# arpitbansal297/Cold-Diffusion-Models

Hardware: NVIDIA H100
Metric: training-step images/sec (CelebA-128 deblur UNet, config 3) (higher is better)
Workload: dtype tf32

## Files before the change

cold_diffusion_models_b200/_lib.py:

```python
import ctypes as C
import os
import torch

_HERE = os.path.dirname(os.path.abspath(__file__))
LIB_PATH = os.path.join(_HERE, 'csrc', 'libcolddiff.so')
CD_MAX_TAPS = 16
CONV_SIMT, CONV_TC = 0, 1
ACT_NONE, ACT_GELU, ACT_GELU_BWD = 0, 1, 2


class ColdDiffError(RuntimeError):
    pass


if not os.path.exists(LIB_PATH):
    raise ImportError("libcolddiff.so not built (%s); run `python -c 'import __graft_entry__ as g; g.build()'`"
                      % LIB_PATH)
lib = C.CDLL(LIB_PATH)


class ConvSrc(C.Structure):
    _fields_ = [('src', C.c_void_p), ('ld', C.c_int32), ('C', C.c_int32), ('H', C.c_int32), ('W', C.c_int32),
                ('ntaps', C.c_int32), ('dy', C.c_int32 * CD_MAX_TAPS), ('dx', C.c_int32 * CD_MAX_TAPS),
                ('w', C.c_void_p), ('w_per_batch', C.c_int32)]


class ConvDesc(C.Structure):
    _fields_ = [('B', C.c_int32), ('Hg', C.c_int32), ('Wg', C.c_int32), ('sy', C.c_int32), ('sx', C.c_int32),
                ('Cout', C.c_int32), ('nsrc', C.c_int32), ('s', ConvSrc * 2),
                ('out', C.c_void_p), ('out_ld', C.c_int32), ('Ho', C.c_int32), ('Wo', C.c_int32),
                ('oys', C.c_int32), ('oxs', C.c_int32), ('oy0', C.c_int32), ('ox0', C.c_int32),
                ('bias', C.c_void_p), ('resid', C.c_void_p), ('resid_ld', C.c_int32),
                ('act', C.c_int32), ('round_tf32', C.c_int32),
                ('out2', C.c_void_p), ('out2_ld', C.c_int32),
                ('aux', C.c_void_p), ('aux_ld', C.c_int32)]




class RepackJob(C.Structure):
    _fields_ = [('src', C.c_void_p), ('dst', C.c_void_p), ('O', C.c_int32), ('I', C.c_int32), ('KH', C.c_int32), ('KW', C.c_int32),
                ('transposed_conv', C.c_int32), ('mode', C.c_int32), ('ntaps', C.c_int32), ('round_tf32', C.c_int32),
                ('ky', C.c_int32 * CD_MAX_TAPS), ('kx', C.c_int32 * CD_MAX_TAPS), ('block0', C.c_int32), ('nblocks', C.c_int32)]


lib.cd_version.restype = C.c_int
if os.environ.get('COLDDIFF_2CTA') in ('0', '1', '2'):
    lib.cd_conv_tc_set_2cta(int(os.environ['COLDDIFF_2CTA']))
lib.cd_last_error.argtypes = [C.c_char_p, C.c_size_t]
if os.environ.get('COLDDIFF_CONV_TWO_CTAS') in ('0', '64', '128', '192'):
    lib.cd_conv_tc_set_two_ctas(int(os.environ['COLDDIFF_CONV_TWO_CTAS']))
if os.environ.get('COLDDIFF_CONV_HALO') in ('0', '1', '2', '6', '8'):
    lib.cd_conv_tc_set_halo(int(os.environ['COLDDIFF_CONV_HALO']))
if os.environ.get('COLDDIFF_WGRAD_MODE') in ('0', '1', '8'):
    lib.cd_wgrad_tc_set_mode(int(os.environ['COLDDIFF_WGRAD_MODE']))
if os.environ.get('COLDDIFF_2CTA_BN') in ('0', '64', '128', '192'):
    lib.cd_conv_tc_set_2cta_bn(int(os.environ['COLDDIFF_2CTA_BN']))
if os.environ.get('COLDDIFF_CONV_STAGED_EPILOGUE') in ('0', '1', '2', '3'):
    lib.cd_conv_tc_set_staged_epilogue(int(os.environ['COLDDIFF_CONV_STAGED_EPILOGUE']))


def _check(rc, what):
    if rc != 0:
        buf = C.create_string_buffer(512)
        lib.cd_last_error(buf, 512)
        raise ColdDiffError("%s failed (%d): %s" % (what, rc, buf.value.decode()))


def stream():
    return C.c_void_p(torch.cuda.current_stream().cuda_stream)


def ptr(t):
    if t is None:
        return C.c_void_p(0)
    return C.c_void_p(t.data_ptr())


_LAUNCHES = {'cd_linattn_context_det': 2, 'cd_conv_wgrad': 2, 'cd_time_mlp_fwd': 2, 'cd_time_mlp2_fwd': 2, 'cd_version': 0, 'cd_last_error': 0}
_launch_count = 0


_PROF_SHAPE_ARGS = {'cd_dwconv7_fwd': (2, 3, 4, 5), 'cd_dwconv7_wgrad': (4, 5, 6, 7), 'cd_layernorm_bwd': (6, 7),
                    'cd_layernorm_fwd': (2, 3), 'cd_linattn_context_det': (2, 3), 'cd_linattn_bwd_kv': (2, 3)}
_prof = None
# ... 47 lines not shown
```

cold_diffusion_models_b200/csrc/conv_tc.cu:

```cuda
#include "tc_common.cuh"
#include "conv_epilogue.cuh"

namespace {

constexpr int kTileM = 128;
constexpr int kChunkK = 32;
constexpr int kABytes = kTileM * 128;
constexpr int kThreads = 288;
constexpr int kConsumerWarps = 8;

struct TcParams {
  int B, Hg, Wg;
  int TW, TH, TN;
  int tiles_x, tiles_y, tiles_n, tiles_co, total_tiles;
  int sy, sx;
  int Cout;
  int nsrc;
  int ntaps[2];
  int kchunks[2];
  int wpb[2];
  int8_t dy[2][CD_MAX_TAPS];
  int8_t dx[2][CD_MAX_TAPS];
  float* out; int out_ld; int Ho, Wo; int oys, oxs, oy0, ox0;
  const float* bias;
// ... 164 lines not shown
            asm volatile("bar.sync %0, 128;" :: "r"(bar_id) : "memory");
            const int w4 = tid >> 5;
            if (w4 < 2) {
              const int row = w4 * 32 + lane;
              uint32_t r[32];
#pragma unroll
              for (int e = 0; e < 32; ++e) r[e] = __float_as_uint(st[row * kEpiStageStride + e]);
              const long long pix = tile_pixel(p, tile, cw * 64 + row);
              cd_epilogue_staged32(r, st + w4 * 32 * kEpiStageStride, lane, pix < 0 ? 0 : pix, pix >= 0, co0 + c, p);
            }
          } else {
#pragma unroll
            for (int j = c / 8; j < c / 8 + 4; ++j) {
              if (pix0 >= 0) epi_pair(p, pix0, co0 + 8 * j + q2, acc[4 * j], acc[4 * j + 1]);
              if (pix1 >= 0) epi_pair(p, pix1, co0 + 8 * j + q2, acc[4 * j + 2], acc[4 * j + 3]);
            }
          }
        }
      } else {
#pragma unroll
        for (int j = 0; j < BN / 8; ++j) {
          if (pix0 >= 0) epi_pair(p, pix0, co0 + 8 * j + q2, acc[4 * j], acc[4 * j + 1]);
          if (pix1 >= 0) epi_pair(p, pix1, co0 + 8 * j + q2, acc[4 * j + 2], acc[4 * j + 3]);
        }
      }
    }
  }
  if constexpr (PAIR) cluster_sync();
}

constexpr int kRowsTW = 16, kRowsTH = kTileM / kRowsTW;
constexpr int kRowsBoxBytes = kRowsTW * (kRowsTH + 2) * 128;

template <int BN, int ABOXES, int STAGES, int CTAS>
__global__ void __launch_bounds__(kThreads, CTAS)
conv_rows_kernel(const __grid_constant__ CUtensorMap mapA0, const __grid_constant__ CUtensorMap mapA1,
                 const __grid_constant__ CUtensorMap mapB0, const __grid_constant__ CUtensorMap mapB1, const __grid_constant__ TcParams p) {
  constexpr int kBBytes = BN * 128;
  extern __shared__ uint8_t smem_raw[];
  const uint32_t raw_addr = smem_u32(smem_raw);
  uint8_t* smem = smem_raw + ((1024u - (raw_addr & 1023u)) & 1023u);
  uint8_t* abox = smem;
  uint8_t* wtile = smem + ABOXES * kRowsBoxBytes;
  uint64_t* bars = reinterpret_cast<uint64_t*>(wtile + STAGES * kBBytes);
  uint64_t* full_bar = bars;
  uint64_t* empty_bar = bars + STAGES;
  uint64_t* afull = bars + 2 * STAGES;
  uint64_t* aempty = bars + 2 * STAGES + ABOXES;
  static_assert(2 * (STAGES + ABOXES) * 8 <= 256, "barrier block is 256 bytes");
  const int warp = threadIdx.x >> 5, lane = threadIdx.x & 31, wg = threadIdx.x >> 7;
  if (threadIdx.x == 0) {
    for (int i = 0; i < STAGES; ++i) { mbar_init(&full_bar[i], 1); mbar_init(&empty_bar[i], kConsumerWarps); }
    for (int i = 0; i < ABOXES; ++i) { mbar_init(&afull[i], 1); mbar_init(&aempty[i], kConsumerWarps); }
    asm volatile("fence.mbarrier_init.release.cluster;" ::: "memory");
  }
  __syncthreads();

  if (warp == kConsumerWarps) {
    if (elect_one()) {
      uint32_t stage = 0, ph = 0, ai = 0, aph = 0;
      for (int tile = blockIdx.x; tile < p.total_tiles; tile += gridDim.x) {
        const int co0 = (tile % p.tiles_co) * BN;
        int mt = tile / p.tiles_co;
        const int x0 = (mt % p.tiles_x) * kRowsTW; mt /= p.tiles_x;
        const int y0 = (mt % p.tiles_y) * kRowsTH;
        const int n = mt / p.tiles_y;
        for (int s = 0; s < p.nsrc; ++s) {
          const CUtensorMap* mA = s ? &mapA1 : &mapA0;
          const CUtensorMap* mB = s ? &mapB1 : &mapB0;
          for (int kc = 0; kc < p.kchunks[s]; ++kc) {
            for (int b = 0, i = 0; b < p.nbox[s]; ++b) {
              mbar_wait(&aempty[ai], aph ^ 1u);
              mbar_expect_tx(&afull[ai], kRowsBoxBytes);
              tma_load_4d(smem_u32(abox + ai * kRowsBoxBytes), mA, &afull[ai], kc * kChunkK, x0 + p.boxdx[s][b], y0 - 1, n);
              if (++ai == ABOXES) { ai = 0; aph ^= 1u; }
              for (; i < p.boxend[s][b]; ++i) {
                mbar_wait(&empty_bar[stage], ph ^ 1u);
                mbar_expect_tx(&full_bar[stage], kBBytes);
                tma_load_3d(smem_u32(wtile + stage * kBBytes), mB, &full_bar[stage], kc * kChunkK, co0, p.taporder[s][i]);
                if (++stage == STAGES) { stage = 0; ph ^= 1u; }
              }
            }
          }
        }
      }
    }
    __syncwarp();
    return;
  }

  const int tid = threadIdx.x & 127;
  const int rl = (tid >> 5) * 16 + (lane >> 2);
  const int q2 = (lane & 3) * 2;
  auto release = [&](uint64_t* bar) { __syncwarp(); if (lane == 0) mbar_arrive(bar); };
  float acc[BN / 2];
  uint32_t stage = 0, ph = 0, ai = 0, aph = 0;
  for (int tile = blockIdx.x; tile < p.total_tiles; tile += gridDim.x) {
    int k = 0;
    uint32_t prev = 0, prev_a = 0;
    for (int s = 0; s < p.nsrc; ++s) {
      for (int kc = 0; kc < p.kchunks[s]; ++kc) {
        for (int b = 0, i = 0; b < p.nbox[s]; ++b) {
          mbar_wait(&afull[ai], aph);
          const uint32_t abase = smem_u32(abox + ai * kRowsBoxBytes) + wg * (kABytes / 2);
          for (const int i0 = i; i < p.boxend[s][b]; ++i, ++k) {
            mbar_wait(&full_bar[stage], ph);
            wgmma_fence();
            const uint64_t da = make_kmajor_sw128_desc(abase + p.tapoff[s][i]);
            const uint64_t db = make_kmajor_sw128_desc(smem_u32(wtile + stage * kBBytes));
#pragma unroll
            for (int kk = 0; kk < 4; ++kk)
              wgmma_tf32<BN>(acc, da + uint64_t(kk * 2), db + uint64_t(kk * 2), (k | kk) != 0 ? 1u : 0u);
            wgmma_commit();
            wgmma_wait<1>();
            if (k > 0) release(&empty_bar[prev]);
            if (k > 0 && i == i0) release(&aempty[prev_a]);
            prev = stage;
            if (++stage == STAGES) { stage = 0; ph ^= 1u; }
          }
          prev_a = ai;
          if (++ai == ABOXES) { ai = 0; aph ^= 1u; }
        }
      }
    }
    wgmma_wait<0>();
    if (k > 0) { release(&empty_bar[prev]); release(&aempty[prev_a]); }

    const int co0 = (tile % p.tiles_co) * BN;
    int mt = tile / p.tiles_co;
    const int x0 = (mt % p.tiles_x) * kRowsTW; mt /= p.tiles_x;
    const int y0 = (mt % p.tiles_y) * kRowsTH;
    const int n = mt / p.tiles_y;
#pragma unroll
    for (int h = 0; h < 2; ++h) {
      const int m = wg * 64 + rl + 8 * h;
      const int gx = x0 + m % kRowsTW, gy = y0 + m / kRowsTW;
      if (gx >= p.Wg || gy >= p.Hg) continue;
      const long long pix = (static_cast<long long>(n) * p.Ho + (gy * p.oys + p.oy0)) * p.Wo + (gx * p.oxs + p.ox0);
#pragma unroll
      for (int j = 0; j < BN / 8; ++j) epi_pair(p, pix, co0 + 8 * j + q2, acc[4 * j + 2 * h], acc[4 * j + 2 * h + 1]);
    }
  }
}


int g_tf32_map_dtype = 1;

template <auto Kernel, size_t kSmem, int CTAS, bool PAIR = false>
int launch_persistent(const CUtensorMap* maps, const TcParams& p, cudaStream_t st) {
  static_assert(kSmem <= 232448, "dynamic shared memory of one CTA (227 KB)");
  static_assert(CTAS == 1 || 2 * (kSmem + 1024) <= 233472, "two CTAs per SM must fit the 228 KB of shared memory");
  CD_CUDA(smem_limit_once<Kernel>(kSmem));
  if constexpr (PAIR) {
    const int units = p.tiles_co * ((p.total_tiles / p.tiles_co + 1) / 2), slots = cd_num_sms() / 2;
    cudaLaunchConfig_t cfg = {};
    cudaLaunchAttribute attr[1];
    attr[0].id = cudaLaunchAttributeClusterDimension;
    attr[0].val.clusterDim.x = 2; attr[0].val.clusterDim.y = 1; attr[0].val.clusterDim.z = 1;
    cfg.gridDim = dim3(2 * (units < slots ? units : slots)); cfg.blockDim = dim3(kThreads);
    cfg.dynamicSmemBytes = kSmem; cfg.stream = st; cfg.attrs = attr; cfg.numAttrs = 1;
    CD_CUDA(cudaLaunchKernelEx(&cfg, Kernel, maps[0], maps[1], maps[2], maps[3], p));
  } else {
    const int slots = cd_num_sms() * CTAS;
    const int grid = p.total_tiles < slots ? p.total_tiles : slots;
    Kernel<<<grid, kThreads, kSmem, st>>>(maps[0], maps[1], maps[2], maps[3], p);
  }
  CD_LAUNCH_CHECK();
  return 0;
}

template <int BN, int STAGES, bool STG = false, bool F16 = false, int CTAS = 1, bool PAIR = false>
int launch(const CUtensorMap* maps, const TcParams& p, cudaStream_t st) {
  constexpr size_t smem = size_t(STAGES) * (kABytes + BN * 128) + 1024 + 256 + (STG ? sizeof(float) * 2 * 64 * kEpiStageStride : 0);
  return launch_persistent<conv_tc_kernel<BN, STAGES, STG, F16, CTAS, PAIR>, smem, CTAS, PAIR>(maps, p, st);
}

template <int BN, int ABOXES, int STAGES, int CTAS = 1>
int launch_rows(const CUtensorMap* maps, const TcParams& p, cudaStream_t st) {
  constexpr size_t smem = size_t(ABOXES) * kRowsBoxBytes + size_t(STAGES) * BN * 128 + 1024 + 256;
  return launch_persistent<conv_rows_kernel<BN, ABOXES, STAGES, CTAS>, smem, CTAS>(maps, p, st);
}

bool operands_ok(const CdConvDesc* d, int chunk_elems, int esz, bool report) {
#define TC_CHECK(cond, ...) do { if (!(cond)) { if (report) cd_set_error(__VA_ARGS__); return false; } } while (0)
  TC_CHECK(d->nsrc >= 1 && d->nsrc <= 2, "conv_tc: nsrc must be 1 or 2");
  TC_CHECK(d->act != CD_ACT_GELU_BWD || (d->aux && (reinterpret_cast<uintptr_t>(d->aux) & 15) == 0 && d->aux_ld % 4 == 0), "conv_tc: GELU_BWD needs an aligned aux");
  TC_CHECK((reinterpret_cast<uintptr_t>(d->out) & 15) == 0 && d->out_ld % 4 == 0, "conv_tc: out must be 16B aligned");
  TC_CHECK(!d->resid || ((reinterpret_cast<uintptr_t>(d->resid) & 15) == 0 && d->resid_ld % 4 == 0), "conv_tc: resid alignment");
  TC_CHECK(!d->out2 || ((reinterpret_cast<uintptr_t>(d->out2) & 15) == 0 && d->out2_ld % 4 == 0), "conv_tc: out2 alignment");
  TC_CHECK(!d->bias || (reinterpret_cast<uintptr_t>(d->bias) & 15) == 0, "conv_tc: bias alignment");
  for (int s = 0; s < d->nsrc; ++s) {
    const CdConvSrc& cs = d->s[s];
    TC_CHECK(cs.C % chunk_elems == 0 && cs.C > 0, "conv_tc: source channels %d not a multiple of %d", cs.C, chunk_elems);
    TC_CHECK(cs.ntaps >= 1 && cs.ntaps <= CD_MAX_TAPS, "conv_tc: bad ntaps");
    TC_CHECK((reinterpret_cast<uintptr_t>(cs.src) & 15) == 0 && (cs.ld * esz) % 16 == 0, "conv_tc: src must be 16B aligned");
    TC_CHECK((reinterpret_cast<uintptr_t>(cs.w) & 15) == 0, "conv_tc: weights must be 16B aligned");
  }
#undef TC_CHECK
  return true;
}

TcParams desc_params(const CdConvDesc* d, int chunk_elems) {
  TcParams p{};
  p.B = d->B; p.Hg = d->Hg; p.Wg = d->Wg; p.sy = d->sy; p.sx = d->sx; p.Cout = d->Cout; p.nsrc = d->nsrc;
  for (int s = 0; s < 2; ++s) {
    const CdConvSrc& cs = d->s[s < d->nsrc ? s : 0];
    p.ntaps[s] = cs.ntaps; p.kchunks[s] = cs.C / chunk_elems; p.wpb[s] = cs.w_per_batch;
    for (int t = 0; t < cs.ntaps; ++t) { p.dy[s][t] = (int8_t)cs.dy[t]; p.dx[s][t] = (int8_t)cs.dx[t]; }
  }
  p.out = d->out; p.out_ld = d->out_ld; p.Ho = d->Ho; p.Wo = d->Wo;
  p.oys = d->oys; p.oxs = d->oxs; p.oy0 = d->oy0; p.ox0 = d->ox0;
  p.bias = d->bias; p.resid = d->resid; p.resid_ld = d->resid_ld; p.act = d->act; p.round_tf32 = d->round_tf32;
  p.out2 = d->out2; p.out2_ld = d->out2_ld; p.aux = d->aux; p.aux_ld = d->aux_ld;
  return p;
}
// ... 3 lines not shown
extern "C" int cd_conv_tc_set_tf32_maps(int enable) { g_tf32_map_dtype = enable ? 1 : 0; return 0; }

static int g_use_2cta = 0;
extern "C" int cd_conv_tc_set_2cta(int mode) { g_use_2cta = mode; return 0; }
static int g_2cta_bn = 0;
extern "C" int cd_conv_tc_set_2cta_bn(int mask) { g_2cta_bn = mask & (128 | 64); return 0; }
static int g_use_halo = 0;
extern "C" int cd_conv_tc_set_halo(int enable) { g_use_halo = enable; return 0; }
static int g_ctas2 = 128 | 64;
extern "C" int cd_conv_tc_set_two_ctas(int mask) { g_ctas2 = mask & (128 | 64); return 0; }
static int g_epi_staged = 0;
constexpr int kStagedMaxKIters = 16;
constexpr int kStagedMidKIters = 48;
extern "C" int cd_conv_tc_set_staged_epilogue(int mode) { g_epi_staged = mode; return 0; }

static double tc_cost(long long m_tiles, int Cout, int BN, int sms, bool pair = false) {
  if (pair) {
    const long long tiles = ((m_tiles + 1) / 2) * (Cout / 256), slots = sms / 2;
    return double((tiles + slots - 1) / slots) * 256.0;
  }
  const long long tiles = m_tiles * ((Cout + BN - 1) / BN);
  const double rate = BN == 256 ? 0.92 : (BN == 128 ? 0.75 : 0.40);
  return double((tiles + sms - 1) / sms) * BN / rate;
}

static int conv_fwd_tc_impl(const CdConvDesc* d, cudaStream_t st, bool f16);
int cd_conv_fwd_tc(const CdConvDesc* d, cudaStream_t st) { return conv_fwd_tc_impl(d, st, false); }

extern "C" int cd_conv_fwd_f16_probe(const CdConvDesc* d, void* stream) {
  CD_REQUIRE(d != nullptr && d->nsrc >= 1 && d->nsrc <= 2, "cd_conv_fwd_f16_probe: bad descriptor");
  return conv_fwd_tc_impl(d, static_cast<cudaStream_t>(stream), true);
}

static int conv_fwd_rows(const CdConvDesc* d, cudaStream_t st, bool by_shape);

static int conv_fwd_tc_impl(const CdConvDesc* d, cudaStream_t st, bool f16) {
  if (!f16 && g_epi_staged == 0) {
    if ((g_use_halo == 0 && !g_use_2cta) || g_use_halo == 1 || g_use_halo == 2 || g_use_halo == 6) {
      const int r = conv_fwd_rows(d, st, g_use_halo == 0);
      if (r <= 0) return r;
    }
  }
  const CUtensorMapDataType dt = f16 ? CU_TENSOR_MAP_DATA_TYPE_FLOAT16 : (g_tf32_map_dtype ? CU_TENSOR_MAP_DATA_TYPE_TFLOAT32 : CU_TENSOR_MAP_DATA_TYPE_FLOAT32);
  const int esz = map_elem_bytes(dt), chunk_elems = 128 / esz;
  if (!operands_ok(d, chunk_elems, esz, true)) return -1;
  TcParams p = desc_params(d, chunk_elems);
  if (d->Wg >= 128) {
    CD_REQUIRE(d->Wg % 128 == 0, "conv_tc: Wg >= 128 must be a multiple of 128 (got %d)", d->Wg);
    p.TW = 128; p.TH = 1; p.TN = 1;
  } else {
    CD_REQUIRE(is_pow2(d->Wg), "conv_tc: Wg < 128 must be a power of two (got %d)", d->Wg);
    p.TW = d->Wg;
    int th = 128 / p.TW;
    if (th > d->Hg) th = d->Hg;
    CD_REQUIRE(is_pow2(th) && d->Hg % th == 0, "conv_tc: unsupported Hg %d for Wg %d", d->Hg, d->Wg);
    p.TH = th; p.TN = 128 / (p.TW * p.TH);
  }
  CD_REQUIRE(p.TW * d->sx <= 256 && p.TH * d->sy <= 256, "conv_tc: strided box too large");
  p.tiles_x = d->Wg / p.TW; p.tiles_y = d->Hg / p.TH; p.tiles_n = cd_cdiv(d->B, p.TN);
  int BN = (d->Cout % 256 == 0) ? 256 : (d->Cout > 64 ? 128 : 64);
  int kiters_host = 0;
  for (int s = 0; s < d->nsrc; ++s) kiters_host += d->s[s].ntaps * (d->s[s].C / chunk_elems);
  const bool staged = !f16 &&
                      ( g_epi_staged == 2 || (g_epi_staged == 1 && kiters_host <= kStagedMaxKIters) ||
                      (g_epi_staged == 3 && kiters_host <= kStagedMidKIters));
  bool pair = false;
  const long long mt = static_cast<long long>(p.tiles_x) * p.tiles_y * p.tiles_n;
  const int sms = cd_num_sms();
  if (BN == 256) {
    double best = tc_cost(mt, d->Cout, 256, sms);
    if (tc_cost(mt, d->Cout, 128, sms) < best) { BN = 128; best = tc_cost(mt, d->Cout, 128, sms); }
    if (!f16 && !staged && g_use_2cta && mt >= 2 && (g_use_2cta == 2 || tc_cost(mt, d->Cout, 256, sms, true) < best)) {
// ... 6 lines not shown
  p.total_tiles = p.tiles_x * p.tiles_y * p.tiles_n * p.tiles_co;

  CUtensorMap maps[4];
  for (int s = 0; s < 2; ++s) {
    const CdConvSrc& cs = d->s[s < d->nsrc ? s : 0];
    CD_REQUIRE(!cs.w_per_batch || p.TN == 1, "conv_tc: per-batch weights need >=128 pixels per image");
    if (!encode_nhwc(&maps[s], dt, cs.src, cs.ld, cs.C, cs.W, cs.H, d->B, 1, 1, 0, 0, p.TW * d->sx, p.TH * d->sy, p.TN, d->sx, d->sy,
                     s ? "A1" : "A0") ||
        !encode_weights(&maps[2 + s], dt, cs.w, cs.C, d->Cout, cs.ntaps * (cs.w_per_batch ? d->B : 1), pair ? BN / 2 : BN,
                        s ? "B1" : "B0"))
      return -1;
  }
  if (f16) {
    if (BN == 256) return launch<256, 4, false, true>(maps, p, st);
    if (BN == 128) return launch<128, 6, false, true>(maps, p, st);
    return launch<64, 8, false, true>(maps, p, st);
  }
  if (staged) {
    if (BN == 256) return launch<256, 3, true>(maps, p, st);
    if (BN == 128) return launch<128, 4, true>(maps, p, st);
    return launch<64, 6, true>(maps, p, st);
  }
  if (pair) {
    if (BN == 256) return launch<256, 4, false, false, 1, true>(maps, p, st);
    if (BN == 128) return launch<128, 6, false, false, 1, true>(maps, p, st);
    return launch<64, 8, false, false, 1, true>(maps, p, st);
  }
  const int ctas2 = p.total_tiles > sms ? g_ctas2 : 0;
  if (BN == 256) return launch<256, 4>(maps, p, st);
  if (BN == 128) return (ctas2 & 128) ? launch<128, 3, false, false, 2>(maps, p, st) : launch<128, 6>(maps, p, st);
  return (ctas2 & 64) ? launch<64, 4, false, false, 2>(maps, p, st) : launch<64, 8>(maps, p, st);
}

static int conv_fwd_rows(const CdConvDesc* d, cudaStream_t st, bool by_shape) {
  if (d->sy != 1 || d->sx != 1 || !operands_ok(d, kChunkK, 4, false)) return 1;
  for (int s = 0; s < d->nsrc; ++s) {
    const CdConvSrc& cs = d->s[s];
    if (cs.w_per_batch || cs.W != d->Wg || cs.H != d->Hg) return 1;
    for (int t = 0; t < cs.ntaps; ++t) if (cs.dy[t] < -1 || cs.dy[t] > 1 || cs.dx[t] < -1 || cs.dx[t] > 1) return 1;
  }
  TcParams p = desc_params(d, kChunkK);
  p.TW = kRowsTW; p.TH = kRowsTH; p.TN = 1;
  p.tiles_x = cd_cdiv(d->Wg, kRowsTW); p.tiles_y = cd_cdiv(d->Hg, kRowsTH); p.tiles_n = d->B;
  const int BN = d->Cout > 64 ? 128 : 64;
  p.tiles_co = cd_cdiv(d->Cout, BN);
  p.total_tiles = p.tiles_x * p.tiles_y * p.tiles_n * p.tiles_co;
  const int sms = cd_num_sms();
  if (by_shape && p.total_tiles <= sms) return 1;
  const CUtensorMapDataType dt = g_tf32_map_dtype ? CU_TENSOR_MAP_DATA_TYPE_TFLOAT32 : CU_TENSOR_MAP_DATA_TYPE_FLOAT32;
  CUtensorMap maps[4];
  for (int s = 0; s < 2; ++s) {
    const CdConvSrc& cs = d->s[s < d->nsrc ? s : 0];
    int i = 0;
    for (int dx = -1; dx <= 1; ++dx) {
      const int i0 = i;
      for (int t = 0; t < cs.ntaps; ++t)
        if (cs.dx[t] == dx) { p.taporder[s][i] = (int8_t)t; p.tapoff[s][i] = (cs.dy[t] + 1) * kRowsTW * 128; ++i; }
      if (i > i0) { p.boxdx[s][p.nbox[s]] = (int8_t)dx; p.boxend[s][p.nbox[s]] = (int8_t)i; ++p.nbox[s]; }
    }
    if (s == 0 && cs.ntaps < 3 * p.nbox[0]) return 1;
    if (!encode_nhwc(&maps[s], dt, cs.src, cs.ld, cs.C, cs.W, cs.H, d->B, 1, 1, 0, 0, kRowsTW, kRowsTH + 2, 1, 1, 1,
                     s ? "rows A1" : "rows A0") ||
        !encode_weights(&maps[2 + s], dt, cs.w, cs.C, d->Cout, cs.ntaps, BN, s ? "rows B1" : "rows B0"))
      return -1;
  }
  const int ctas2 = p.total_tiles > sms ? g_ctas2 : 0;
  if (BN == 128) return (ctas2 & 128) ? launch_rows<128, 3, 3, 2>(maps, p, st) : launch_rows<128, 6, 4>(maps, p, st);
  return (ctas2 & 64) ? launch_rows<64, 3, 6, 2>(maps, p, st) : launch_rows<64, 6, 8>(maps, p, st);
}
```

cold_diffusion_models_b200/csrc/dwconv_tma.cu:

```cuda
#include "tc_common.cuh"

namespace {

constexpr int kTY = 16;
constexpr int kWTX = 16;

__device__ __forceinline__ float* align128(uint8_t* raw) {
  return reinterpret_cast<float*>(raw + ((128u - (smem_u32(raw) & 127u)) & 127u));
}
__device__ __forceinline__ void fence_proxy_async() { asm volatile("fence.proxy.async.shared::cta;" ::: "memory"); }

template <int TX>
__global__ void __launch_bounds__(32 * kTY, 1)
dwconv7_tma_kernel(const __grid_constant__ CUtensorMap mapX, int B, int H, int W, int C,
                   const float* __restrict__ wdw, const float* __restrict__ bdw, const float* __restrict__ cond, int cond_ld,
                   float* __restrict__ out, int out_ld, int flip, const float* __restrict__ addend, int addend_ld) {
  extern __shared__ uint8_t dw_smem_raw[];
  float* xsp = align128(dw_smem_raw);
  __shared__ uint64_t full[2];
  constexpr int TY = kTY, XW = TX + 6, YH = TY + 6;
  constexpr int tile_floats = YH * XW * 32;
  const int lane = threadIdx.x & 31, ry = threadIdx.x >> 5;
  const int tiles_x = W / TX, tiles_y = H / TY;
  const int ntiles = B * tiles_x * tiles_y;
  const int total = (C / 32) * ntiles;

  if (threadIdx.x == 0) {
    mbar_init(&full[0], 1); mbar_init(&full[1], 1);
    asm volatile("fence.mbarrier_init.release.cluster;" ::: "memory");
  }
  __syncthreads();

  auto issue = [&](int item, int bi) {
    const int slab = item / ntiles, t = item - slab * ntiles;
    const int tx = t % tiles_x, ty = (t / tiles_x) % tiles_y, b = t / (tiles_x * tiles_y);
    fence_proxy_async();
    mbar_expect_tx(&full[bi], tile_floats * 4);
    tma_load_4d(smem_u32(xsp + bi * tile_floats), &mapX, &full[bi], slab * 32, tx * TX - 3, ty * TY - 3, b);
  };

  int item = blockIdx.x;
  if (item >= total) return;
  int bufi = 0;
// ... 182 lines not shown
```

cold_diffusion_models_b200/csrc/tc_common.cuh:

```cuda
#pragma once
#include "cd_common.cuh"

namespace {

__device__ __forceinline__ uint32_t smem_u32(const void* p) {
  return static_cast<uint32_t>(__cvta_generic_to_shared(p));
}
__device__ __forceinline__ uint32_t elect_one() {
  uint32_t pred = 0;
  asm volatile(
      "{\n"
      ".reg .pred px;\n"
      "elect.sync _|px, 0xffffffff;\n"
      "@px mov.s32 %0, 1;\n"
      "}\n" : "+r"(pred));
  return pred;
}
__device__ __forceinline__ void mbar_init(uint64_t* bar, uint32_t count) {
  asm volatile("mbarrier.init.shared::cta.b64 [%0], %1;" :: "r"(smem_u32(bar)), "r"(count) : "memory");
}
__device__ __forceinline__ void mbar_expect_tx(uint64_t* bar, uint32_t bytes) {
  asm volatile("mbarrier.arrive.expect_tx.shared::cta.b64 _, [%0], %1;"
               :: "r"(smem_u32(bar)), "r"(bytes) : "memory");
}
__device__ __forceinline__ void mbar_arrive(uint64_t* bar) {
  asm volatile("mbarrier.arrive.shared::cta.b64 _, [%0];" :: "r"(smem_u32(bar)) : "memory");
}
__device__ __forceinline__ void mbar_wait(uint64_t* bar, uint32_t parity) {
  asm volatile(
      "{\n"
      ".reg .pred p;\n"
      "WAIT_%=:\n"
      "mbarrier.try_wait.parity.shared::cta.b64 p, [%0], %1;\n"
      "@p bra DONE_%=;\n"
      "bra WAIT_%=;\n"
      "DONE_%=:\n"
      "}\n" :: "r"(smem_u32(bar)), "r"(parity) : "memory");
}
__device__ __forceinline__ void tma_load_4d(uint32_t dst, const CUtensorMap* map, uint64_t* bar,
                                            int c0, int c1, int c2, int c3) {
  asm volatile(
      "cp.async.bulk.tensor.4d.shared::cluster.global.mbarrier::complete_tx::bytes"
      " [%0], [%1, {%3, %4, %5, %6}], [%2];"
      :: "r"(dst), "l"(reinterpret_cast<uint64_t>(map)), "r"(smem_u32(bar)),
         "r"(c0), "r"(c1), "r"(c2), "r"(c3) : "memory");
}
__device__ __forceinline__ void tma_load_3d(uint32_t dst, const CUtensorMap* map, uint64_t* bar,
                                            int c0, int c1, int c2) {
  asm volatile(
      "cp.async.bulk.tensor.3d.shared::cluster.global.mbarrier::complete_tx::bytes"
      " [%0], [%1, {%3, %4, %5}], [%2];"
      :: "r"(dst), "l"(reinterpret_cast<uint64_t>(map)), "r"(smem_u32(bar)),
         "r"(c0), "r"(c1), "r"(c2) : "memory");
}
__device__ __forceinline__ uint64_t make_kmajor_sw128_desc(uint32_t saddr) {
  uint64_t d = 0;
  d |= static_cast<uint64_t>((saddr >> 4) & 0x3FFFu);
  d |= static_cast<uint64_t>(1) << 16;
  d |= static_cast<uint64_t>(1024 >> 4) << 32;
  d |= static_cast<uint64_t>(1) << 62;
  return d;
}
__device__ __forceinline__ void wgmma_fence() { asm volatile("wgmma.fence.sync.aligned;" ::: "memory"); }
__device__ __forceinline__ void wgmma_commit() { asm volatile("wgmma.commit_group.sync.aligned;" ::: "memory"); }
template <int N>
__device__ __forceinline__ void wgmma_wait() { asm volatile("wgmma.wait_group.sync.aligned %0;" :: "n"(N) : "memory"); }

template <int N> __device__ __forceinline__ void wgmma_tf32(float (&d)[N / 2], uint64_t da, uint64_t db, uint32_t acc);
template <int N> __device__ __forceinline__ void wgmma_f16(float (&d)[N / 2], uint64_t da, uint64_t db, uint32_t acc);
template <> __device__ __forceinline__ void wgmma_tf32<64>(float (&d)[32], uint64_t da, uint64_t db, uint32_t acc) {
  asm volatile(
      "{\n.reg .pred p;\nsetp.ne.b32 p, %34, 0;\n"
      "wgmma.mma_async.sync.aligned.m64n64k8.f32.tf32.tf32 {%0, %1, %2, %3, %4, %5, %6, %7, %8, %9, %10, %11, %12, %13, %14, %15, %16, %17, %18, %19, %20, %21, %22, %23, %24, %25, %26, %27, %28, %29, %30, %31}, %32, %33, p, 1, 1;\n}\n"
      : "+f"(d[0]), "+f"(d[1]), "+f"(d[2]), "+f"(d[3]), "+f"(d[4]), "+f"(d[5]), "+f"(d[6]), "+f"(d[7]), "+f"(d[8]), "+f"(d[9]), "+f"(d[10]), "+f"(d[11]), "+f"(d[12]), "+f"(d[13]), "+f"(d[14]), "+f"(d[15]), "+f"(d[16]), "+f"(d[17]), "+f"(d[18]), "+f"(d[19]), "+f"(d[20]), "+f"(d[21]), "+f"(d[22]), "+f"(d[23]), "+f"(d[24]), "+f"(d[25]), "+f"(d[26]), "+f"(d[27]), "+f"(d[28]), "+f"(d[29]), "+f"(d[30]), "+f"(d[31])
      : "l"(da), "l"(db), "r"(acc));
}
template <> __device__ __forceinline__ void wgmma_tf32<128>(float (&d)[64], uint64_t da, uint64_t db, uint32_t acc) {
  asm volatile(
      "{\n.reg .pred p;\nsetp.ne.b32 p, %66, 0;\n"
      "wgmma.mma_async.sync.aligned.m64n128k8.f32.tf32.tf32 {%0, %1, %2, %3, %4, %5, %6, %7, %8, %9, %10, %11, %12, %13, %14, %15, %16, %17, %18, %19, %20, %21, %22, %23, %24, %25, %26, %27, %28, %29, %30, %31, %32, %33, %34, %35, %36, %37, %38, %39, %40, %41, %42, %43, %44, %45, %46, %47, %48, %49, %50, %51, %52, %53, %54, %55, %56, %57, %58, %59, %60, %61, %62, %63}, %64, %65, p, 1, 1;\n}\n"
      : "+f"(d[0]), "+f"(d[1]), "+f"(d[2]), "+f"(d[3]), "+f"(d[4]), "+f"(d[5]), "+f"(d[6]), "+f"(d[7]), "+f"(d[8]), "+f"(d[9]), "+f"(d[10]), "+f"(d[11]), "+f"(d[12]), "+f"(d[13]), "+f"(d[14]), "+f"(d[15]), "+f"(d[16]), "+f"(d[17]), "+f"(d[18]), "+f"(d[19]), "+f"(d[20]), "+f"(d[21]), "+f"(d[22]), "+f"(d[23]), "+f"(d[24]), "+f"(d[25]), "+f"(d[26]), "+f"(d[27]), "+f"(d[28]), "+f"(d[29]), "+f"(d[30]), "+f"(d[31]), "+f"(d[32]), "+f"(d[33]), "+f"(d[34]), "+f"(d[35]), "+f"(d[36]), "+f"(d[37]), "+f"(d[38]), "+f"(d[39]), "+f"(d[40]), "+f"(d[41]), "+f"(d[42]), "+f"(d[43]), "+f"(d[44]), "+f"(d[45]), "+f"(d[46]), "+f"(d[47]), "+f"(d[48]), "+f"(d[49]), "+f"(d[50]), "+f"(d[51]), "+f"(d[52]), "+f"(d[53]), "+f"(d[54]), "+f"(d[55]), "+f"(d[56]), "+f"(d[57]), "+f"(d[58]), "+f"(d[59]), "+f"(d[60]), "+f"(d[61]), "+f"(d[62]), "+f"(d[63])
      : "l"(da), "l"(db), "r"(acc));
}
template <> __device__ __forceinline__ void wgmma_tf32<256>(float (&d)[128], uint64_t da, uint64_t db, uint32_t acc) {
  asm volatile(
      "{\n.reg .pred p;\nsetp.ne.b32 p, %130, 0;\n"
      "wgmma.mma_async.sync.aligned.m64n256k8.f32.tf32.tf32 {%0, %1, %2, %3, %4, %5, %6, %7, %8, %9, %10, %11, %12, %13, %14, %15, %16, %17, %18, %19, %20, %21, %22, %23, %24, %25, %26, %27, %28, %29, %30, %31, %32, %33, %34, %35, %36, %37, %38, %39, %40, %41, %42, %43, %44, %45, %46, %47, %48, %49, %50, %51, %52, %53, %54, %55, %56, %57, %58, %59, %60, %61, %62, %63, %64, %65, %66, %67, %68, %69, %70, %71, %72, %73, %74, %75, %76, %77, %78, %79, %80, %81, %82, %83, %84, %85, %86, %87, %88, %89, %90, %91, %92, %93, %94, %95, %96, %97, %98, %99, %100, %101, %102, %103, %104, %105, %106, %107, %108, %109, %110, %111, %112, %113, %114, %115, %116, %117, %118, %119, %120, %121, %122, %123, %124, %125, %126, %127}, %128, %129, p, 1, 1;\n}\n"
// ... 129 lines not shown
```

Before: 622.1.

## Add 256-pixel rows conv kernel with two consumer warpgroups and TMA-store epilogue

Adds a conv_rows256 kernel that uses a taller 16x16 pixel tile, so each loaded halo box is shared by two consumer warpgroups, each issuing two 64-row wgmma accumulators. It uses setmaxnreg to shift registers from the producer warpgroup to the consumers, and writes results through swizzled shared-memory staging and TMA bulk stores. The kernel is chosen by default when the taller tiling still gives enough tiles to fill the SMs and the output is unstrided. This is meant to cut A-operand reload traffic per output and the cost of scattered global stores, at the price of fewer tiles (possible SM underfill) and one CTA per SM. The producer loop is refactored into a shared helper.

```diff
diff --git a/cold_diffusion_models_b200/_lib.py b/cold_diffusion_models_b200/_lib.py
--- a/cold_diffusion_models_b200/_lib.py
+++ b/cold_diffusion_models_b200/_lib.py
@@ -50,7 +50,7 @@
 lib.cd_last_error.argtypes = [C.c_char_p, C.c_size_t]
 if os.environ.get('COLDDIFF_CONV_TWO_CTAS') in ('0', '64', '128', '192'):
     lib.cd_conv_tc_set_two_ctas(int(os.environ['COLDDIFF_CONV_TWO_CTAS']))
-if os.environ.get('COLDDIFF_CONV_HALO') in ('0', '1', '2', '6', '8'):
+if os.environ.get('COLDDIFF_CONV_HALO') in ('0', '1', '2', '4', '6', '8'):
     lib.cd_conv_tc_set_halo(int(os.environ['COLDDIFF_CONV_HALO']))
 if os.environ.get('COLDDIFF_WGRAD_MODE') in ('0', '1', '8'):
     lib.cd_wgrad_tc_set_mode(int(os.environ['COLDDIFF_WGRAD_MODE']))
diff --git a/cold_diffusion_models_b200/csrc/conv_tc.cu b/cold_diffusion_models_b200/csrc/conv_tc.cu
--- a/cold_diffusion_models_b200/csrc/conv_tc.cu
+++ b/cold_diffusion_models_b200/csrc/conv_tc.cu
@@ -220,6 +220,43 @@
 constexpr int kRowsTW = 16, kRowsTH = kTileM / kRowsTW;
 constexpr int kRowsBoxBytes = kRowsTW * (kRowsTH + 2) * 128;
 
+template <int BN, int TH, int ABOXES, int STAGES>
+__device__ __forceinline__ void rows_producer(const CUtensorMap& mapA0, const CUtensorMap& mapA1, const CUtensorMap& mapB0,
+                                              const CUtensorMap& mapB1, const TcParams& p, uint8_t* abox, uint8_t* wtile,
+                                              uint64_t* afull, uint64_t* aempty, uint64_t* full_bar, uint64_t* empty_bar) {
+  constexpr int kBBytes = BN * 128;
+  constexpr int kBoxBytes = kRowsTW * (TH + 2) * 128;
+  if (elect_one()) {
+    uint32_t stage = 0, ph = 0, ai = 0, aph = 0;
+    for (int tile = blockIdx.x; tile < p.total_tiles; tile += gridDim.x) {
+      const int co0 = (tile % p.tiles_co) * BN;
+      int mt = tile / p.tiles_co;
+      const int x0 = (mt % p.tiles_x) * kRowsTW; mt /= p.tiles_x;
+      const int y0 = (mt % p.tiles_y) * TH;
+      const int n = mt / p.tiles_y;
+      for (int s = 0; s < p.nsrc; ++s) {
+        const CUtensorMap* mA = s ? &mapA1 : &mapA0;
+        const CUtensorMap* mB = s ? &mapB1 : &mapB0;
+        for (int kc = 0; kc < p.kchunks[s]; ++kc) {
+          for (int b = 0, i = 0; b < p.nbox[s]; ++b) {
+            mbar_wait(&aempty[ai], aph ^ 1u);
+            mbar_expect_tx(&afull[ai], kBoxBytes);
+            tma_load_4d(smem_u32(abox + ai * kBoxBytes), mA, &afull[ai], kc * kChunkK, x0 + p.boxdx[s][b], y0 - 1, n);
+            if (++ai == ABOXES) { ai = 0; aph ^= 1u; }
+            for (; i < p.boxend[s][b]; ++i) {
+              mbar_wait(&empty_bar[stage], ph ^ 1u);
+              mbar_expect_tx(&full_bar[stage], kBBytes);
+              tma_load_3d(smem_u32(wtile + stage * kBBytes), mB, &full_bar[stage], kc * kChunkK, co0, p.taporder[s][i]);
+              if (++stage == STAGES) { stage = 0; ph ^= 1u; }
+            }
+          }
+        }
+      }
+    }
+  }
+  __syncwarp();
+}
+
 template <int BN, int ABOXES, int STAGES, int CTAS>
 __global__ void __launch_bounds__(kThreads, CTAS)
 conv_rows_kernel(const __grid_constant__ CUtensorMap mapA0, const __grid_constant__ CUtensorMap mapA1,
@@ -245,35 +282,7 @@
   __syncthreads();
 
   if (warp == kConsumerWarps) {
-    if (elect_one()) {
-      uint32_t stage = 0, ph = 0, ai = 0, aph = 0;
-      for (int tile = blockIdx.x; tile < p.total_tiles; tile += gridDim.x) {
-        const int co0 = (tile % p.tiles_co) * BN;
-        int mt = tile / p.tiles_co;
-        const int x0 = (mt % p.tiles_x) * kRowsTW; mt /= p.tiles_x;
-        const int y0 = (mt % p.tiles_y) * kRowsTH;
-        const int n = mt / p.tiles_y;
-        for (int s = 0; s < p.nsrc; ++s) {
-          const CUtensorMap* mA = s ? &mapA1 : &mapA0;
-          const CUtensorMap* mB = s ? &mapB1 : &mapB0;
-          for (int kc = 0; kc < p.kchunks[s]; ++kc) {
-            for (int b = 0, i = 0; b < p.nbox[s]; ++b) {
-              mbar_wait(&aempty[ai], aph ^ 1u);
-              mbar_expect_tx(&afull[ai], kRowsBoxBytes);
-              tma_load_4d(smem_u32(abox + ai * kRowsBoxBytes), mA, &afull[ai], kc * kChunkK, x0 + p.boxdx[s][b], y0 - 1, n);
-              if (++ai == ABOXES) { ai = 0; aph ^= 1u; }
-              for (; i < p.boxend[s][b]; ++i) {
-                mbar_wait(&empty_bar[stage], ph ^ 1u);
-                mbar_expect_tx(&full_bar[stage], kBBytes);
-                tma_load_3d(smem_u32(wtile + stage * kBBytes), mB, &full_bar[stage], kc * kChunkK, co0, p.taporder[s][i]);
-                if (++stage == STAGES) { stage = 0; ph ^= 1u; }
-              }
-            }
-          }
-        }
-      }
-    }
-    __syncwarp();
+    rows_producer<BN, kRowsTH, ABOXES, STAGES>(mapA0, mapA1, mapB0, mapB1, p, abox, wtile, afull, aempty, full_bar, empty_bar);
     return;
   }
 
@@ -331,6 +340,193 @@
   }
 }
 
+constexpr int kR256TH = 16;
+constexpr int kR256BoxBytes = kRowsTW * (kR256TH + 2) * 128;
+constexpr int kR256Slice = 128 * 128;
+constexpr int kR256Threads = 384;
+constexpr int kR256RegsLow = 40, kR256RegsHigh = 232;
+
+__device__ __forceinline__ float2 ld_pair(const float* row, int col, int Cout, bool ok) {
+  if (ok && col + 1 < Cout) return *reinterpret_cast<const float2*>(row + col);
+  if (ok && col < Cout) return make_float2(row[col], 0.f);
+  return make_float2(0.f, 0.f);
+}
+
+template <int BN, int ABOXES, int STAGES>
+__global__ void __launch_bounds__(kR256Threads, 1)
+conv_rows256_kernel(const __grid_constant__ CUtensorMap mapA0, const __grid_constant__ CUtensorMap mapA1,
+                    const __grid_constant__ CUtensorMap mapB0, const __grid_constant__ CUtensorMap mapB1,
+                    const __grid_constant__ CUtensorMap mapO, const __grid_constant__ CUtensorMap mapO2, const __grid_constant__ TcParams p) {
+  constexpr int kBBytes = BN * 128;
+  extern __shared__ uint8_t smem_raw[];
+  const uint32_t raw_addr = smem_u32(smem_raw);
+  uint8_t* smem = smem_raw + ((1024u - (raw_addr & 1023u)) & 1023u);
+  uint8_t* abox = smem;
+  uint8_t* wtile = smem + ABOXES * kR256BoxBytes;
+  uint8_t* stg = wtile + STAGES * kBBytes;
+  uint64_t* bars = reinterpret_cast<uint64_t*>(stg + 4 * kR256Slice);
+  uint64_t* full_bar = bars;
+  uint64_t* empty_bar = bars + STAGES;
+  uint64_t* afull = bars + 2 * STAGES;
+  uint64_t* aempty = bars + 2 * STAGES + ABOXES;
+  static_assert(2 * (STAGES + ABOXES) * 8 <= 256, "barrier block is 256 bytes");
+  const int warp = threadIdx.x >> 5, lane = threadIdx.x & 31, wg = threadIdx.x >> 7;
+  if (threadIdx.x == 0) {
+    for (int i = 0; i < STAGES; ++i) { mbar_init(&full_bar[i], 1); mbar_init(&empty_bar[i], kConsumerWarps); }
+    for (int i = 0; i < ABOXES; ++i) { mbar_init(&afull[i], 1); mbar_init(&aempty[i], kConsumerWarps); }
+    asm volatile("fence.mbarrier_init.release.cluster;" ::: "memory");
+  }
+  __syncthreads();
+
+  if (wg == 0) {
+    asm volatile("setmaxnreg.dec.sync.aligned.u32 %0;" :: "n"(kR256RegsLow));
+    if (warp == 0)
+      rows_producer<BN, kR256TH, ABOXES, STAGES>(mapA0, mapA1, mapB0, mapB1, p, abox, wtile, afull, aempty, full_bar, empty_bar);
+    return;
+  }
+  asm volatile("setmaxnreg.inc.sync.aligned.u32 %0;" :: "n"(kR256RegsHigh));
+
+  const int cw = wg - 1;
+  const int tid = threadIdx.x & 127;
+  const int rl = (tid >> 5) * 16 + (lane >> 2);
+  const int q2 = (lane & 3) * 2;
+  const bool storer = tid == 0;
+  uint8_t* so = stg + cw * 2 * kR256Slice;
+  uint8_t* so2 = so + kR256Slice;
+  auto release = [&](uint64_t* bar) { __syncwarp(); if (lane == 0) mbar_arrive(bar); };
+  auto wg_sync = [&]() { asm volatile("bar.sync %0, 128;" :: "r"(1 + cw) : "memory"); };
+  float acc[2][BN / 2];
+  uint32_t stage = 0, ph = 0, ai = 0, aph = 0;
+  for (int tile = blockIdx.x; tile < p.total_tiles; tile += gridDim.x) {
+    int k = 0;
+    uint32_t prev = 0, prev_a = 0;
+    for (int s = 0; s < p.nsrc; ++s) {
+      for (int kc = 0; kc < p.kchunks[s]; ++kc) {
+        for (int b = 0, i = 0; b < p.nbox[s]; ++b) {
+          mbar_wait(&afull[ai], aph);
+          const uint32_t abase = smem_u32(abox + ai * kR256BoxBytes) + cw * kABytes;
+          for (const int i0 = i; i < p.boxend[s][b]; ++i, ++k) {
+            mbar_wait(&full_bar[stage], ph);
+            wgmma_fence();
+            const uint64_t da0 = make_kmajor_sw128_desc(abase + p.tapoff[s][i]);
+            const uint64_t da1 = make_kmajor_sw128_desc(abase + p.tapoff[s][i] + kABytes / 2);
+            const uint64_t db = make_kmajor_sw128_desc(smem_u32(wtile + stage * kBBytes));
+#pragma unroll
+            for (int kk = 0; kk < 4; ++kk) {
+              wgmma_tf32<BN>(acc[0], da0 + uint64_t(kk * 2), db + uint64_t(kk * 2), (k | kk) != 0 ? 1u : 0u);
+              wgmma_tf32<BN>(acc[1], da1 + uint64_t(kk * 2), db + uint64_t(kk * 2), (k | kk) != 0 ? 1u : 0u);
+            }
+            wgmma_commit();
+            wgmma_wait<1>();
+            if (k > 0) release(&empty_bar[prev]);
+            if (k > 0 && i == i0) release(&aempty[prev_a]);
+            prev = stage;
+            if (++stage == STAGES) { stage = 0; ph ^= 1u; }
+          }
+          prev_a = ai;
+          if (++ai == ABOXES) { ai = 0; aph ^= 1u; }
+        }
+      }
+    }
+    wgmma_wait<0>();
+    if (k > 0) { release(&empty_bar[prev]); release(&aempty[prev_a]); }
+
+    const int co0 = (tile % p.tiles_co) * BN;
+    int mt = tile / p.tiles_co;
+    const int x0 = (mt % p.tiles_x) * kRowsTW; mt /= p.tiles_x;
+    const int yw = (mt % p.tiles_y) * kR256TH + 8 * cw;
+    const int n = mt / p.tiles_y;
+    if (yw >= p.Hg) continue;
+    long long pix[2][2];
+    bool valid[2][2];
+#pragma unroll
+    for (int h = 0; h < 2; ++h)
+#pragma unroll
+      for (int e = 0; e < 2; ++e) {
+        const int r = 64 * h + rl + 8 * e, gx = x0 + r % kRowsTW, gy = yw + r / kRowsTW;
+        valid[h][e] = gx < p.Wg && gy < p.Hg;
+        pix[h][e] = (static_cast<long long>(n) * p.Hg + gy) * p.Wg + gx;
+      }
+#pragma unroll
+    for (int c = 0; c < BN / 32; ++c) {
+      if (co0 + 32 * c >= p.Cout) break;
+      if (storer) bulk_wait_read<0>();
+      wg_sync();
+#pragma unroll
+      for (int h = 0; h < 2; ++h) {
+        float2 v[2][4];
+#pragma unroll
+        for (int e = 0; e < 2; ++e)
+#pragma unroll
+          for (int jj = 0; jj < 4; ++jj) v[e][jj] = make_float2(acc[h][16 * c + 4 * jj + 2 * e], acc[h][16 * c + 4 * jj + 2 * e + 1]);
+        if (p.bias) {
+#pragma unroll
+          for (int jj = 0; jj < 4; ++jj) {
+            const float2 b = ld_pair(p.bias, co0 + 32 * c + 8 * jj + q2, p.Cout, true);
+#pragma unroll
+            for (int e = 0; e < 2; ++e) { v[e][jj].x += b.x; v[e][jj].y += b.y; }
+          }
+        }
+        if (p.resid) {
+          float2 r[2][4];
+#pragma unroll
+          for (int e = 0; e < 2; ++e)
+#pragma unroll
+            for (int jj = 0; jj < 4; ++jj) r[e][jj] = ld_pair(p.resid + pix[h][e] * p.resid_ld, co0 + 32 * c + 8 * jj + q2, p.Cout, valid[h][e]);
+#pragma unroll
+          for (int e = 0; e < 2; ++e)
+#pragma unroll
+            for (int jj = 0; jj < 4; ++jj) { v[e][jj].x += r[e][jj].x; v[e][jj].y += r[e][jj].y; }
+        }
+        auto soff = [&](int e, int jj) {
+          const int rr = 64 * h + rl + 8 * e;
+          return rr * 128 + ((((8 * jj + q2) >> 2) ^ (rr & 7)) << 4) + (q2 & 3) * 4;
+        };
+        if (p.out2) {
+#pragma unroll
+          for (int e = 0; e < 2; ++e)
+#pragma unroll
+            for (int jj = 0; jj < 4; ++jj) *reinterpret_cast<float2*>(so2 + soff(e, jj)) = v[e][jj];
+        }
+        if (p.act == CD_ACT_GELU) {
+#pragma unroll
+          for (int e = 0; e < 2; ++e)
+#pragma unroll
+            for (int jj = 0; jj < 4; ++jj) { v[e][jj].x = cd_gelu(v[e][jj].x); v[e][jj].y = cd_gelu(v[e][jj].y); }
+        } else if (p.act == CD_ACT_GELU_BWD) {
+          float2 a[2][4];
+#pragma unroll
+          for (int e = 0; e < 2; ++e)
+#pragma unroll
+            for (int jj = 0; jj < 4; ++jj) a[e][jj] = ld_pair(p.aux + pix[h][e] * p.aux_ld, co0 + 32 * c + 8 * jj + q2, p.Cout, valid[h][e]);
+#pragma unroll
+          for (int e = 0; e < 2; ++e)
+#pragma unroll
+            for (int jj = 0; jj < 4; ++jj) { v[e][jj].x *= cd_gelu_grad(a[e][jj].x); v[e][jj].y *= cd_gelu_grad(a[e][jj].y); }
+        }
+        if (p.round_tf32) {
+#pragma unroll
+          for (int e = 0; e < 2; ++e)
+#pragma unroll
+            for (int jj = 0; jj < 4; ++jj) { v[e][jj].x = cd_round_tf32(v[e][jj].x); v[e][jj].y = cd_round_tf32(v[e][jj].y); }
+        }
+#pragma unroll
+        for (int e = 0; e < 2; ++e)
+#pragma unroll
+          for (int jj = 0; jj < 4; ++jj) *reinterpret_cast<float2*>(so + soff(e, jj)) = v[e][jj];
+      }
+      fence_proxy_async();
+      wg_sync();
+      if (storer) {
+        tma_store_4d(&mapO, smem_u32(so), co0 + 32 * c, x0, yw, n);
+        if (p.out2) tma_store_4d(&mapO2, smem_u32(so2), co0 + 32 * c, x0, yw, n);
+        bulk_commit();
+      }
+    }
+  }
+  if (storer) bulk_wait<0>();
+}
+
 
 int g_tf32_map_dtype = 1;
 
@@ -369,6 +565,19 @@
   return launch_persistent<conv_rows_kernel<BN, ABOXES, STAGES, CTAS>, smem, CTAS>(maps, p, st);
 }
 
+template <int BN, int ABOXES, int STAGES>
+int launch_rows256(const CUtensorMap* maps, const TcParams& p, cudaStream_t st) {
+  constexpr size_t smem = size_t(ABOXES) * kR256BoxBytes + size_t(STAGES) * BN * 128 + 4 * kR256Slice + 1024 + 256;
+  static_assert(smem <= 232448, "dynamic shared memory of one CTA (227 KB)");
+  constexpr auto kernel = conv_rows256_kernel<BN, ABOXES, STAGES>;
+  CD_CUDA(smem_limit_once<kernel>(smem));
+  const int sms = cd_num_sms();
+  const int grid = p.total_tiles < sms ? p.total_tiles : sms;
+  kernel<<<grid, kR256Threads, smem, st>>>(maps[0], maps[1], maps[2], maps[3], maps[4], maps[5], p);
+  CD_LAUNCH_CHECK();
+  return 0;
+}
+
 bool operands_ok(const CdConvDesc* d, int chunk_elems, int esz, bool report) {
 #define TC_CHECK(cond, ...) do { if (!(cond)) { if (report) cd_set_error(__VA_ARGS__); return false; } } while (0)
   TC_CHECK(d->nsrc >= 1 && d->nsrc <= 2, "conv_tc: nsrc must be 1 or 2");
@@ -438,12 +647,12 @@
   return conv_fwd_tc_impl(d, static_cast<cudaStream_t>(stream), true);
 }
 
-static int conv_fwd_rows(const CdConvDesc* d, cudaStream_t st, bool by_shape);
+static int conv_fwd_rows(const CdConvDesc* d, cudaStream_t st, int mode);
 
 static int conv_fwd_tc_impl(const CdConvDesc* d, cudaStream_t st, bool f16) {
   if (!f16 && g_epi_staged == 0) {
-    if ((g_use_halo == 0 && !g_use_2cta) || g_use_halo == 1 || g_use_halo == 2 || g_use_halo == 6) {
-      const int r = conv_fwd_rows(d, st, g_use_halo == 0);
+    if ((g_use_halo == 0 && !g_use_2cta) || g_use_halo == 1 || g_use_halo == 2 || g_use_halo == 4 || g_use_halo == 6) {
+      const int r = conv_fwd_rows(d, st, g_use_halo);
       if (r <= 0) return r;
     }
   }
@@ -516,7 +725,8 @@
   return (ctas2 & 64) ? launch<64, 4, false, false, 2>(maps, p, st) : launch<64, 8>(maps, p, st);
 }
 
-static int conv_fwd_rows(const CdConvDesc* d, cudaStream_t st, bool by_shape) {
+static int conv_fwd_rows(const CdConvDesc* d, cudaStream_t st, int mode) {
+  const bool by_shape = mode == 0;
   if (d->sy != 1 || d->sx != 1 || !operands_ok(d, kChunkK, 4, false)) return 1;
   for (int s = 0; s < d->nsrc; ++s) {
     const CdConvSrc& cs = d->s[s];
@@ -531,8 +741,12 @@
   p.total_tiles = p.tiles_x * p.tiles_y * p.tiles_n * p.tiles_co;
   const int sms = cd_num_sms();
   if (by_shape && p.total_tiles <= sms) return 1;
+  const int tiles256 = p.tiles_x * cd_cdiv(d->Hg, kR256TH) * p.tiles_n * p.tiles_co;
+  const bool rows256 = (mode == 4 || (by_shape && 4 * tiles256 >= 3 * sms)) && d->oys == 1 && d->oxs == 1 && d->oy0 == 0 &&
+                       d->ox0 == 0 && d->Ho == d->Hg && d->Wo == d->Wg;
+  if (rows256) { p.TH = kR256TH; p.tiles_y = cd_cdiv(d->Hg, kR256TH); p.total_tiles = tiles256; }
   const CUtensorMapDataType dt = g_tf32_map_dtype ? CU_TENSOR_MAP_DATA_TYPE_TFLOAT32 : CU_TENSOR_MAP_DATA_TYPE_FLOAT32;
-  CUtensorMap maps[4];
+  CUtensorMap maps[6];
   for (int s = 0; s < 2; ++s) {
     const CdConvSrc& cs = d->s[s < d->nsrc ? s : 0];
     int i = 0;
@@ -543,11 +757,22 @@
       if (i > i0) { p.boxdx[s][p.nbox[s]] = (int8_t)dx; p.boxend[s][p.nbox[s]] = (int8_t)i; ++p.nbox[s]; }
     }
     if (s == 0 && cs.ntaps < 3 * p.nbox[0]) return 1;
-    if (!encode_nhwc(&maps[s], dt, cs.src, cs.ld, cs.C, cs.W, cs.H, d->B, 1, 1, 0, 0, kRowsTW, kRowsTH + 2, 1, 1, 1,
+    if (!encode_nhwc(&maps[s], dt, cs.src, cs.ld, cs.C, cs.W, cs.H, d->B, 1, 1, 0, 0, kRowsTW, p.TH + 2, 1, 1, 1,
                      s ? "rows A1" : "rows A0") ||
         !encode_weights(&maps[2 + s], dt, cs.w, cs.C, d->Cout, cs.ntaps, BN, s ? "rows B1" : "rows B0"))
       return -1;
   }
+  if (rows256) {
+    const float* o2 = d->out2 ? d->out2 : d->out;
+    const int o2ld = d->out2 ? d->out2_ld : d->out_ld;
+    if (!encode_nhwc(&maps[4], CU_TENSOR_MAP_DATA_TYPE_FLOAT32, d->out, d->out_ld, d->Cout, d->Wg, d->Hg, d->B, 1, 1, 0, 0, kRowsTW,
+                     kR256TH / 2, 1, 1, 1, "rows out") ||
+        !encode_nhwc(&maps[5], CU_TENSOR_MAP_DATA_TYPE_FLOAT32, o2, o2ld, d->Cout, d->Wg, d->Hg, d->B, 1, 1, 0, 0, kRowsTW,
+                     kR256TH / 2, 1, 1, 1, "rows out2"))
+      return -1;
+    if (BN == 128) return launch_rows256<128, 3, 3>(maps, p, st);
+    return launch_rows256<64, 3, 6>(maps, p, st);
+  }
   const int ctas2 = p.total_tiles > sms ? g_ctas2 : 0;
   if (BN == 128) return (ctas2 & 128) ? launch_rows<128, 3, 3, 2>(maps, p, st) : launch_rows<128, 6, 4>(maps, p, st);
   return (ctas2 & 64) ? launch_rows<64, 3, 6, 2>(maps, p, st) : launch_rows<64, 6, 8>(maps, p, st);
diff --git a/cold_diffusion_models_b200/csrc/dwconv_tma.cu b/cold_diffusion_models_b200/csrc/dwconv_tma.cu
--- a/cold_diffusion_models_b200/csrc/dwconv_tma.cu
+++ b/cold_diffusion_models_b200/csrc/dwconv_tma.cu
@@ -8,7 +8,6 @@
 __device__ __forceinline__ float* align128(uint8_t* raw) {
   return reinterpret_cast<float*>(raw + ((128u - (smem_u32(raw) & 127u)) & 127u));
 }
-__device__ __forceinline__ void fence_proxy_async() { asm volatile("fence.proxy.async.shared::cta;" ::: "memory"); }
 
 template <int TX>
 __global__ void __launch_bounds__(32 * kTY, 1)
diff --git a/cold_diffusion_models_b200/csrc/tc_common.cuh b/cold_diffusion_models_b200/csrc/tc_common.cuh
--- a/cold_diffusion_models_b200/csrc/tc_common.cuh
+++ b/cold_diffusion_models_b200/csrc/tc_common.cuh
@@ -53,6 +53,16 @@
       :: "r"(dst), "l"(reinterpret_cast<uint64_t>(map)), "r"(smem_u32(bar)),
          "r"(c0), "r"(c1), "r"(c2) : "memory");
 }
+__device__ __forceinline__ void fence_proxy_async() { asm volatile("fence.proxy.async.shared::cta;" ::: "memory"); }
+__device__ __forceinline__ void tma_store_4d(const CUtensorMap* map, uint32_t src, int c0, int c1, int c2, int c3) {
+  asm volatile("cp.async.bulk.tensor.4d.global.shared::cta.bulk_group [%0, {%2, %3, %4, %5}], [%1];"
+               :: "l"(reinterpret_cast<uint64_t>(map)), "r"(src), "r"(c0), "r"(c1), "r"(c2), "r"(c3) : "memory");
+}
+__device__ __forceinline__ void bulk_commit() { asm volatile("cp.async.bulk.commit_group;" ::: "memory"); }
+template <int N>
+__device__ __forceinline__ void bulk_wait_read() { asm volatile("cp.async.bulk.wait_group.read %0;" :: "n"(N) : "memory"); }
+template <int N>
+__device__ __forceinline__ void bulk_wait() { asm volatile("cp.async.bulk.wait_group %0;" :: "n"(N) : "memory"); }
 __device__ __forceinline__ uint64_t make_kmajor_sw128_desc(uint32_t saddr) {
   uint64_t d = 0;
   d |= static_cast<uint64_t>((saddr >> 4) & 0x3FFFu);
```

Result: faster. 685.2, median of 6 (+10.1%).
